# pmeletis/IV2019-boosting-semantic-segmentation-with-weak-labels

Measured on NVIDIA B200. Metric: train_images_per_s, higher is better.
Workload: dtype bf16

## Files before the change

### iv2019-boosting-semantic-segmentation-with-weak-labels_b200/csrc/conv_igemm_sm100.cu

```cuda
#include <cuda.h>

#include <cstdlib>
#include <map>
#include <mutex>
#include <tuple>
#include <vector>

#include "common.cuh"
#include "tc_sm100.cuh"

namespace wlseg {

int check_conv_params(const wlseg_conv_params* p);
int conv_fprop_direct(const wlseg_conv_params* p, const void* x, const void* w, void* y, const float* scale,
                      const float* shift, const void* residual, cudaStream_t s);

constexpr int kBM = 128;
constexpr int kBK = 64;
constexpr int kUmmaK = 16;
constexpr int kEpiWarp0 = 4;
constexpr int kABytes = kBM * kBK * 2;
constexpr int kSmemBudget = 224 * 1024;

struct IgemmParams {
  CUtensorMap map_a;
  CUtensorMap map_b;
  CUtensorMap map_y;
  CUtensorMap map_r;
  void* y;
  const float* scale;
  const float* shift;
  const void* res;
  double* bn_sum;
  double* bn_sqsum;
  const uint32_t* out_mask;
  const float* bnb_scale;
  const float* bnb_shift;
  const float* bnb_mean;
  const float* bnb_invstd;
  wlseg_bn_finalize_args fin;
  CUtensorMap map_ah;
  int halo_rows, halo_bytes, halo_sbo;
  int epi_split;
  int N, P, Q, K, C;
  int R, S, stride, dilation, pad_top, pad_left;
  int y_pitch, res_pitch, res_stride, res_H, res_W;
  int relu;
  int tw_log2;
  int tiles_w, tiles_h, n_tiles, total_tiles;
  int cchunks;
  int num_kb;
  int stages;
  int epi_bufs;
  int res_mid;
  int epi_db;
  int reverse;
  FastDiv fd_n_tiles, fd_tiles_w, fd_tiles_h;
  int m_tiles;
  int units;
};

constexpr int kSubW = 64;
constexpr int kWarpBufBytes = 32 * kSubW * 2;
constexpr int kMaxStages = 8;
constexpr int kMaxEpiWarps = 16;
constexpr int kBarBytes = 512;
constexpr int kSmemMax = 227 * 1024;

template <int BN, bool kPair = false>
struct IgemmCfg {
  static constexpr int kBRows = kPair ? BN / 2 : BN;
  static constexpr int kBBytes = kBRows * kBK * 2;
  static constexpr int kStageBytes = kABytes + kBBytes;
  static constexpr int kTmemCols = 2 * BN < 32 ? 32 : 2 * BN;
};

__device__ __forceinline__ void warp_column_sums(float (&v)[32], int lane) {
#pragma unroll
  for (int off = 16; off >= 1; off >>= 1) {
    const bool upper = (lane & off) != 0;
#pragma unroll
    for (int i = 0; i < off; ++i) {
      const float send = upper ? v[i] : v[i + off];
      const float keep = upper ? v[i + off] : v[i];
      v[i] = keep + __shfl_xor_sync(0xffffffffu, send, off);
    }
  }
}

struct SubTileCursor {
  int tile, st;
  int n, p0, q0, k0;
};

template <int BN, bool kPair>
__device__ __forceinline__ void decode_tile(const IgemmParams& prm, int tile, int rank, int& n, int& p0, int& q0, int& k0) {
  uint32_t umt, unt;
  prm.fd_n_tiles.divmod((uint32_t)tile, umt, unt);
  int mt = (int)umt;
  if (kPair) mt = 2 * mt + rank;
  k0 = (int)unt * BN;
  if (kPair && mt >= prm.m_tiles) {
    n = prm.N; p0 = 0; q0 = 0;
    return;
  }
  if (prm.reverse) mt = prm.m_tiles - 1 - mt;
  uint32_t rest, twi, un, thi;
  prm.fd_tiles_w.divmod((uint32_t)mt, rest, twi);
  prm.fd_tiles_h.divmod(rest, un, thi);
  n = (int)un;
  q0 = (int)twi << prm.tw_log2;
  p0 = (int)thi * (kBM >> prm.tw_log2);
}

template <int BN>
__device__ __forceinline__ int num_subtiles(const IgemmParams& prm, int k0) {
  const int left = prm.K - k0;
  const int full = BN / kSubW;
  const int need = (left + kSubW - 1) / kSubW;
  return need < full ? need : full;
}

template <int BN, typename TY, bool kTmaEpi, int EW, bool kPair, bool kBnb = false, bool kHalo = false>
__global__ void __launch_bounds__(128 + 32 * EW, 1)
conv_igemm_kernel(const __grid_constant__ IgemmParams prm) {
  using Cfg = IgemmCfg<BN, kPair>;
  const uint32_t rank = kPair ? cluster_ctarank() : 0u;
  const int unit0 = kPair ? (int)(blockIdx.x >> 1) : (int)blockIdx.x;
  const int unit_step = kPair ? (int)(gridDim.x >> 1) : (int)gridDim.x;
  constexpr int CG = EW / 4;
  extern __shared__ __align__(1024) uint8_t smem[];
  pdl_launch_dependents();
  if ((smem_u32(smem) & 1023u) != 0) __trap();
  const int stages = prm.stages;
  uint8_t* halo_b = smem + 2 * prm.halo_bytes;
  uint8_t* epi_smem = kHalo ? halo_b + prm.num_kb * Cfg::kBBytes : smem + stages * Cfg::kStageBytes;
  uint64_t* bars = reinterpret_cast<uint64_t*>(epi_smem + prm.epi_bufs * kWarpBufBytes);
  uint64_t* full_bar = bars;
  uint64_t* empty_bar = bars + kMaxStages;
  uint64_t* tfull_bar = bars + 2 * kMaxStages;
  uint64_t* tempty_bar = bars + 2 * kMaxStages + 2;
  uint64_t* rfull_bar = bars + 2 * kMaxStages + 4;
  uint32_t* tmem_slot = reinterpret_cast<uint32_t*>(bars + 2 * kMaxStages + 4 + 2 * kMaxEpiWarps);
  uint64_t* afull_bar = bars + 2 * kMaxStages + 4 + 2 * kMaxEpiWarps + 1;
  uint64_t* aempty_bar = afull_bar + 2;
  uint64_t* bfull_bar = afull_bar + 4;
  float* s_stat = reinterpret_cast<float*>(reinterpret_cast<uint8_t*>(bars) + kBarBytes);

  const int warp = threadIdx.x >> 5;
  const int lane = threadIdx.x & 31;

  if (warp == 0 && lane == 0) {
    tma_prefetch_desc(kHalo ? &prm.map_ah : &prm.map_a);
    tma_prefetch_desc(&prm.map_b);
    if (kTmaEpi) {
      tma_prefetch_desc(&prm.map_y);
      if (prm.res != nullptr) tma_prefetch_desc(&prm.map_r);
    }
  }
  if (warp == 1 && lane == 0) {
    for (int s = 0; s < stages; ++s) {
      mbar_init(smem_u32(full_bar + s), 1);
      mbar_init(smem_u32(empty_bar + s), 1);
    }
    for (int a = 0; a < 2; ++a) {
      mbar_init(smem_u32(tfull_bar + a), 1);
      mbar_init(smem_u32(tempty_bar + a), kPair ? 2 * EW : EW);
    }
    for (int a = 0; a < 2 * EW; ++a) mbar_init(smem_u32(rfull_bar + a), 1);
    if (kHalo) {
      for (int a = 0; a < 2; ++a) { mbar_init(smem_u32(afull_bar + a), 1); mbar_init(smem_u32(aempty_bar + a), 1); }
      mbar_init(smem_u32(bfull_bar), 1);
    }
    fence_barrier_init();
  }
  if (warp == 2) {
    if (kPair) tmem_alloc_pair(smem_u32(tmem_slot), Cfg::kTmemCols);
    else tmem_alloc(smem_u32(tmem_slot), Cfg::kTmemCols);
  }
  if (kTmaEpi && warp == 3 && prm.bn_sum != nullptr)
    for (int j = lane; j < 2 * BN; j += 32) s_stat[j] = 0.f;
  tc_fence_before();
  __syncthreads();
  if (kPair) cluster_sync();
  tc_fence_after();
  const uint32_t tmem_base = *tmem_slot;
  pdl_wait();

  const int TW = 1 << prm.tw_log2;

  if (warp == 0) {
    if (kHalo && lane == 0) {
      mbar_arrive_expect_tx(smem_u32(bfull_bar), prm.num_kb * Cfg::kBBytes);
      for (int kb = 0; kb < prm.num_kb; ++kb)
        tma_load_3d(smem_u32(halo_b + kb * Cfg::kBBytes), &prm.map_b, smem_u32(bfull_bar), 0, kb, 0);
      int it = 0;
      for (int tile = unit0; tile < prm.units; tile += unit_step, ++it) {
        int n, p0, q0, k0;
        decode_tile<BN, kPair>(prm, tile, rank, n, p0, q0, k0);
        const int ab = it & 1;
        mbar_wait(smem_u32(aempty_bar + ab), ((uint32_t)(it >> 1) & 1u) ^ 1u);
        mbar_arrive_expect_tx(smem_u32(afull_bar + ab), prm.halo_bytes);
        tma_load_4d(smem_u32(smem + ab * prm.halo_bytes), &prm.map_ah, smem_u32(afull_bar + ab), 0, q0 - prm.pad_left,
                    p0 - prm.pad_top, n);
      }
    } else if (lane == 0) {
      int stage = 0;
      uint32_t phase = 0;
      for (int tile = unit0; tile < prm.units; tile += unit_step) {
        int n, p0, q0, k0;
// ... 41 lines not shown
        for (int kb = 0; kb < prm.num_kb; ++kb) {
          const uint64_t adesc = make_smem_desc_shifted(a_base + (uint32_t)(r * 2048 + sx * 128), (uint32_t)prm.halo_sbo);
          const uint64_t bdesc = make_smem_desc(smem_u32(halo_b + kb * Cfg::kBBytes));
#pragma unroll
          for (int k = 0; k < kBK / kUmmaK; ++k)
            umma_bf16(d_tmem, adesc + (uint64_t)(k * 2), bdesc + (uint64_t)(k * 2), idesc, (kb | k) != 0);
          if (++sx == prm.S) { sx = 0; ++r; }
        }
        umma_commit(smem_u32(aempty_bar + ab));
        umma_commit(smem_u32(tfull_bar + acc));
      }
    } else if (lane == 0 && rank == 0) {
      constexpr uint32_t idesc = make_idesc(kPair ? 2 * kBM : kBM, BN);
      int stage = 0;
      uint32_t phase = 0;
      int iter = 0;
      for (int tile = unit0; tile < prm.units; tile += unit_step, ++iter) {
        const int acc = iter & 1;
        const uint32_t acc_phase = (iter >> 1) & 1;
        mbar_wait(smem_u32(tempty_bar + acc), acc_phase ^ 1);
        tc_fence_after();
        const uint32_t d_tmem = tmem_base + acc * BN;
        for (int kb = 0; kb < prm.num_kb; ++kb) {
          mbar_wait(smem_u32(full_bar + stage), phase);
          tc_fence_after();
          const uint32_t a_addr = smem_u32(smem + stage * Cfg::kStageBytes);
          const uint64_t adesc = make_smem_desc(a_addr);
          const uint64_t bdesc = make_smem_desc(a_addr + kABytes);
#pragma unroll
          for (int k = 0; k < kBK / kUmmaK; ++k) {
            if (kPair) umma_bf16_pair(d_tmem, adesc + (uint64_t)(k * 2), bdesc + (uint64_t)(k * 2), idesc, (kb | k) != 0);
            else umma_bf16(d_tmem, adesc + (uint64_t)(k * 2), bdesc + (uint64_t)(k * 2), idesc, (kb | k) != 0);
          }
          if (kPair) umma_commit_pair(smem_u32(empty_bar + stage), 3); else umma_commit(smem_u32(empty_bar + stage));
          if (++stage == stages) { stage = 0; phase ^= 1; }
        }
        if (kPair) umma_commit_pair(smem_u32(tfull_bar + acc), 3); else umma_commit(smem_u32(tfull_bar + acc));
      }
    }
  } else if (warp >= kEpiWarp0) {
    const int ew = warp - kEpiWarp0;
    const int quarter = ew & 3;
    const int cgrp = ew >> 2;
    const int et = threadIdx.x - kEpiWarp0 * 32;
    const int row = quarter * 32 + lane;
    const int dy_ = row >> prm.tw_log2, dx_ = row & (TW - 1);
    const uint32_t lane_addr = tmem_base + ((uint32_t)(quarter * 32) << 16);
    auto release_acc = [&](int a) {
      if (kPair) mbar_arrive_cluster(mapa_shared(smem_u32(tempty_bar + a), 0));
      else mbar_arrive(smem_u32(tempty_bar + a));
    };
    int iter = 0;
    if constexpr (kTmaEpi) {
      const bool has_res = prm.res != nullptr;
      const bool has_stat = prm.bn_sum != nullptr;
      const uint32_t sw = (uint32_t)(lane & 7);
      const bool dbuf = has_res || prm.epi_db;
      const bool split = BN == kSubW && prm.epi_split != 0;
      uint8_t* wbuf = epi_smem + ((kHalo && !split) ? quarter : ew) * (kBnb ? 3 : (dbuf ? 2 : 1)) * kWarpBufBytes;
      const int st0 = split ? 0 : cgrp;
      const int st_step = split ? BN / kSubW : CG;
      const int tile0 = unit0 + (split ? cgrp * unit_step : 0);
      const int tile_step = split ? 2 * unit_step : unit_step;
      uint64_t* my_rfull = rfull_bar + 2 * ew;
      const int r0 = quarter * 32;
      const int dy0 = r0 >> prm.tw_log2, dx0 = r0 & (TW - 1);
      constexpr int kResPf = 4;
      struct ResCursor { int tile, st, cnt; };
      ResCursor ld = {tile0, st0, 0}, pf = {tile0, st0, 0};
      auto next_residual = [&](ResCursor& c, bool stage) {
        while (c.tile < prm.units) {
          int n, p0, q0, k0;
          decode_tile<BN, kPair>(prm, c.tile, rank, n, p0, q0, k0);
          if (c.st < num_subtiles<BN>(prm, k0)) {
            const int cx = (q0 + dx0) * prm.res_stride, cy = (p0 + dy0) * prm.res_stride;
            if (stage) {
              const uint32_t bar = smem_u32(my_rfull + (c.cnt & 1));
              mbar_arrive_expect_tx(bar, kWarpBufBytes);
              tma_load_4d(smem_u32(wbuf + (c.cnt & 1) * kWarpBufBytes), &prm.map_r, bar, k0 + c.st * kSubW, cx, cy, n);
            } else {
              tma_prefetch_4d(&prm.map_r, k0 + c.st * kSubW, cx, cy, n);
            }
            ++c.cnt;
            c.st += st_step;
            return;
          }
          c.st = st0;
          c.tile += tile_step;
        }
      };
      if (has_res && lane == 0) {
        for (int i = 0; i < kResPf; ++i) next_residual(pf, false);
        next_residual(ld, true);
      }
      constexpr int kSlots = (BN / kSubW + CG - 1) / CG;
      float a1x[kSlots], a1y[kSlots], a2x[kSlots], a2y[kSlots];
#pragma unroll
      for (int i = 0; i < kSlots; ++i) a1x[i] = a1y[i] = a2x[i] = a2y[i] = 0.f;
      int stat_k0 = -1;
      int cnt = 0;
      float bmx[kSlots], bmy[kSlots], bix[kSlots], biy[kSlots];
#pragma unroll
      for (int i = 0; i < kSlots; ++i) bmx[i] = bmy[i] = bix[i] = biy[i] = 0.f;
      uint2 mcur[kSlots], mnext[kSlots];
      auto load_mask = [&](int tile_, uint2 (&m)[kSlots]) {
#pragma unroll
        for (int i = 0; i < kSlots; ++i) m[i] = make_uint2(0xffffffffu, 0xffffffffu);
        if (prm.out_mask == nullptr || tile_ >= prm.units) return;
        int n_, p0_, q0_, k0_;
        decode_tile<BN, kPair>(prm, tile_, rank, n_, p0_, q0_, k0_);
        const bool ok = (p0_ + dy_ < prm.P) && (q0_ + dx_ < prm.Q) && (n_ < prm.N);
        const int nsub_ = num_subtiles<BN>(prm, k0_);
        const uint2* row = reinterpret_cast<const uint2*>(
            prm.out_mask + (((int64_t)n_ * prm.P + p0_ + dy_) * prm.Q + q0_ + dx_) * (prm.K >> 5) + (k0_ >> 5));
#pragma unroll
        for (int i = 0; i < kSlots; ++i) {
          const int st_ = st0 + i * st_step;
          m[i] = (ok && st_ < nsub_) ? __ldg(row + st_) : make_uint2(0u, 0u);
        }
      };
      load_mask(unit0, mnext);
      for (int tile = unit0; tile < prm.units; tile += unit_step, ++iter) {
        int n, p0, q0, k0;
        decode_tile<BN, kPair>(prm, tile, rank, n, p0, q0, k0);
        const bool valid = (p0 + dy_ < prm.P) && (q0 + dx_ < prm.Q) && (n < prm.N);
#pragma unroll
        for (int i = 0; i < kSlots; ++i) mcur[i] = mnext[i];
        load_mask(tile + unit_step, mnext);
        const int acc = iter & 1;
        const uint32_t acc_phase = (iter >> 1) & 1;
        const int nsub = num_subtiles<BN>(prm, k0);
        if (has_stat) {
          if (stat_k0 >= 0 && k0 != stat_k0) __trap();
          if constexpr (kBnb) {
            if (stat_k0 < 0) {
#pragma unroll
              for (int i = 0; i < kSlots; ++i) {
                const int c = k0 + (st0 + i * st_step) * kSubW + 2 * lane;
                if (c + 1 < prm.K) {
                  bmx[i] = __ldg(prm.bnb_mean + c); bmy[i] = __ldg(prm.bnb_mean + c + 1);
                  bix[i] = __ldg(prm.bnb_invstd + c); biy[i] = __ldg(prm.bnb_invstd + c + 1);
                }
              }
            }
          }
          stat_k0 = k0;
        }
        mbar_wait(smem_u32(tfull_bar + acc), acc_phase);
        tc_fence_after();
        const bool idle = split ? ((iter & 1) != cgrp) : (cgrp >= nsub);
        if (idle) {
          tc_fence_before();
          __syncwarp();
          if (lane == 0) release_acc(acc);
        }
#pragma unroll
        for (int slot = 0; slot < kSlots; ++slot) {
          const int st = st0 + slot * st_step;
          if (st >= nsub || idle) break;
          if constexpr (kBnb) {
            uint8_t* zb = wbuf + (cnt & 1) * kWarpBufBytes;
            uint8_t* ob = wbuf + 2 * kWarpBufBytes;
            if (lane == 0) {
              bulk_wait_read<0>();
              next_residual(ld, true);
              next_residual(pf, false);
            }
            __syncwarp();
            mbar_wait(smem_u32(my_rfull + (cnt & 1)), (uint32_t)((cnt >> 1) & 1));
#pragma unroll
            for (int half = 0; half < 2; ++half) {
              const int col = st * kSubW + half * 32;
              uint32_t v[32];
              tmem_ld<32>(lane_addr + (uint32_t)(acc * BN + col), v);
              tmem_ld_wait();
              if (half == 1 && st + CG >= nsub) {
                tc_fence_before();
                __syncwarp();
// ... 4 lines not shown
              for (int j = 0; j < 32; ++j) f[j] = valid ? __uint_as_float(v[j]) : 0.f;
              uint4 raw[4];
#pragma unroll
              for (int g = 0; g < 4; ++g)
                raw[g] = *reinterpret_cast<const uint4*>(zb + lane * 128 + ((((uint32_t)(half * 4 + g)) ^ sw) << 4));
              const float4* sc4 = reinterpret_cast<const float4*>(prm.bnb_scale + k0 + col);
              const float4* sh4 = reinterpret_cast<const float4*>(prm.bnb_shift + k0 + col);
              uint4 outv[4];
#pragma unroll
              for (int g = 0; g < 4; ++g) {
                const __nv_bfloat162* hz = reinterpret_cast<const __nv_bfloat162*>(&raw[g]);
                __nv_bfloat162* ho = reinterpret_cast<__nv_bfloat162*>(&outv[g]);
                const float4 sca = __ldg(sc4 + 2 * g), scb = __ldg(sc4 + 2 * g + 1);
                const float4 sha = __ldg(sh4 + 2 * g), shb = __ldg(sh4 + 2 * g + 1);
                const float scs[8] = {sca.x, sca.y, sca.z, sca.w, scb.x, scb.y, scb.z, scb.w};
                const float shs[8] = {sha.x, sha.y, sha.z, sha.w, shb.x, shb.y, shb.z, shb.w};
#pragma unroll
                for (int e = 0; e < 4; ++e) {
                  const float2 zz = __bfloat1622float2(hz[e]);
                  const float gx = fmaf(zz.x, scs[2 * e], shs[2 * e]) > 0.f ? f[g * 8 + 2 * e] : 0.f;
                  const float gy = fmaf(zz.y, scs[2 * e + 1], shs[2 * e + 1]) > 0.f ? f[g * 8 + 2 * e + 1] : 0.f;
                  ho[e] = __floats2bfloat162_rn(gx, gy);
                }
              }
#pragma unroll
              for (int g = 0; g < 4; ++g)
                *reinterpret_cast<uint4*>(ob + lane * 128 + ((((uint32_t)(half * 4 + g)) ^ sw) << 4)) = outv[g];
            }
            fence_async_smem();
            __syncwarp();
            if (lane == 0) {
              tma_store_4d(&prm.map_y, smem_u32(ob), k0 + st * kSubW, q0 + dx0, p0 + dy0, n);
              bulk_commit();
            }
            {
              const uint32_t coff = (uint32_t)((lane & 3) << 2);
              float s0x = 0.f, s0y = 0.f, s1x = 0.f, s1y = 0.f;
              const float mx = bmx[slot], my = bmy[slot], ix = bix[slot], iy = biy[slot];
#pragma unroll
              for (int r = 0; r < 32; ++r) {
                const uint32_t o = (uint32_t)(r * 128) + ((((uint32_t)(lane >> 2)) ^ (uint32_t)(r & 7)) << 4) + coff;
                const float2 g2 = __bfloat1622float2(*reinterpret_cast<const __nv_bfloat162*>(ob + o));
                const float2 z2 = __bfloat1622float2(*reinterpret_cast<const __nv_bfloat162*>(zb + o));
                s0x += g2.x * (z2.x - mx) * ix; s0y += g2.y * (z2.y - my) * iy;
                s1x += g2.x; s1y += g2.y;
              }
              a1x[slot] += s0x; a1y[slot] += s0y; a2x[slot] += s1x; a2y[slot] += s1y;
            }
            __syncwarp();
            ++cnt;
            continue;
          }
          uint8_t* buf = wbuf + (dbuf ? (cnt & 1) * kWarpBufBytes : 0);
          const bool mid = has_res && prm.res_mid;
          if (lane == 0 && !mid) {
            if (!has_res && dbuf) bulk_wait_read<1>(); else bulk_wait_read<0>();
            if (has_res) {
              next_residual(ld, true);
              next_residual(pf, false);
            }
          }
          __syncwarp();
          if (has_res && !mid) mbar_wait(smem_u32(my_rfull + (cnt & 1)), (uint32_t)((cnt >> 1) & 1));
          uint8_t* myrow = buf + lane * 128;
#pragma unroll
          for (int half = 0; half < 2; ++half) {
            const int col = st * kSubW + half * 32;
            if (mid && half == 1) {
              if (lane == 0) {
                bulk_wait_read<0>();
                next_residual(ld, true);
                next_residual(pf, false);
              }
              __syncwarp();
            }
            const uint32_t mword = half == 0 ? mcur[slot].x : mcur[slot].y;
            uint32_t v[32];
            tmem_ld<32>(lane_addr + (uint32_t)(acc * BN + col), v);
            tmem_ld_wait();
            if (half == 1 && st + CG >= nsub) {
              tc_fence_before();
              __syncwarp();
              if (lane == 0) release_acc(acc);
            }
            float f[32];
#pragma unroll
            for (int j = 0; j < 32; ++j) f[j] = __uint_as_float(v[j]);
            if (prm.scale != nullptr) {
              const float4* sc4 = reinterpret_cast<const float4*>(prm.scale + k0 + col);
              const float4* sh4 = reinterpret_cast<const float4*>(prm.shift + k0 + col);
#pragma unroll
              for (int g = 0; g < 8; ++g) {
                const float4 sc = __ldg(sc4 + g);
                const float4 sh = __ldg(sh4 + g);
                f[g * 4 + 0] = fmaf(f[g * 4 + 0], sc.x, sh.x);
                f[g * 4 + 1] = fmaf(f[g * 4 + 1], sc.y, sh.y);
                f[g * 4 + 2] = fmaf(f[g * 4 + 2], sc.z, sh.z);
                f[g * 4 + 3] = fmaf(f[g * 4 + 3], sc.w, sh.w);
              }
            }
            uint4* slot4[4];
#pragma unroll
            for (int g = 0; g < 4; ++g)
              slot4[g] = reinterpret_cast<uint4*>(myrow + ((((uint32_t)(half * 4 + g)) ^ sw) << 4));
            if (mid && half == 0) mbar_wait(smem_u32(my_rfull + (cnt & 1)), (uint32_t)((cnt >> 1) & 1));
            if (has_res) {
              uint4 raw[4];
#pragma unroll
              for (int g = 0; g < 4; ++g) raw[g] = *slot4[g];
#pragma unroll
              for (int g = 0; g < 4; ++g) {
                const __nv_bfloat162* h = reinterpret_cast<const __nv_bfloat162*>(&raw[g]);
#pragma unroll
                for (int e = 0; e < 4; ++e) {
                  const float2 t = __bfloat1622float2(h[e]);
                  f[g * 8 + 2 * e] += t.x;
                  f[g * 8 + 2 * e + 1] += t.y;
                }
              }
            }
            if (prm.out_mask != nullptr) {
#pragma unroll
              for (int j = 0; j < 32; ++j) f[j] = ((mword >> j) & 1u) ? f[j] : 0.f;
            }
            if (has_stat && !valid) {
#pragma unroll
              for (int j = 0; j < 32; ++j) f[j] = 0.f;
            }
            uint4 outv[4];
            if (prm.relu) {
#pragma unroll
              for (int g = 0; g < 4; ++g) {
                __nv_bfloat162* ho = reinterpret_cast<__nv_bfloat162*>(&outv[g]);
#pragma unroll
                for (int e = 0; e < 4; ++e) {
                  uint32_t packed;
                  asm("cvt.rn.relu.bf16x2.f32 %0, %1, %2;" : "=r"(packed) : "f"(f[g * 8 + 2 * e + 1]), "f"(f[g * 8 + 2 * e]));
                  reinterpret_cast<uint32_t*>(ho)[e] = packed;
                }
              }
            } else {
#pragma unroll
              for (int g = 0; g < 4; ++g) {
                __nv_bfloat162* ho = reinterpret_cast<__nv_bfloat162*>(&outv[g]);
#pragma unroll
                for (int e = 0; e < 4; ++e) ho[e] = __floats2bfloat162_rn(f[g * 8 + 2 * e], f[g * 8 + 2 * e + 1]);
              }
            }
#pragma unroll
            for (int g = 0; g < 4; ++g) *slot4[g] = outv[g];
          }
          fence_async_smem();
          __syncwarp();
          if (lane == 0) {
            tma_store_4d(&prm.map_y, smem_u32(buf), k0 + st * kSubW, q0 + dx0, p0 + dy0, n);
            bulk_commit();
          }
          if (has_stat) {
            const uint8_t* base = buf + ((lane & 3) << 2);
            float s1x = 0.f, s1y = 0.f, s2x = 0.f, s2y = 0.f;
#pragma unroll
            for (int r = 0; r < 32; ++r) {
              const __nv_bfloat162 h = *reinterpret_cast<const __nv_bfloat162*>(
                  base + r * 128 + ((((uint32_t)(lane >> 2)) ^ (uint32_t)(r & 7)) << 4));
              const float2 t = __bfloat1622float2(h);
              s1x += t.x; s1y += t.y;
              s2x = fmaf(t.x, t.x, s2x); s2y = fmaf(t.y, t.y, s2y);
            }
            a1x[slot] += s1x; a1y[slot] += s1y; a2x[slot] += s2x; a2y[slot] += s2y;
          }
          ++cnt;
        }
      }
      if (has_stat) {
        constexpr int kBufsPerWarp = kBnb ? 3 : 0;
        const int nbuf = kBufsPerWarp ? kBufsPerWarp : (dbuf ? 2 : 1);
        if (lane == 0) bulk_wait_read<0>();
        __syncwarp();
        float* park = reinterpret_cast<float*>(wbuf);
#pragma unroll
        for (int i = 0; i < kSlots; ++i) {
          if (kHalo && !split && cgrp != 0) break;
          park[(i * 2 + 0) * kSubW + 2 * lane] = a1x[i]; park[(i * 2 + 0) * kSubW + 2 * lane + 1] = a1y[i];
          park[(i * 2 + 1) * kSubW + 2 * lane] = a2x[i]; park[(i * 2 + 1) * kSubW + 2 * lane + 1] = a2y[i];
        }
        epi_barrier<32 * EW>();
        if (stat_k0 >= 0) {
          for (int j = et; j < BN; j += 32 * EW) {
            if (stat_k0 + j < prm.K) {
              const int st = j / kSubW, ch = j % kSubW;
              const int cg = split ? 0 : st % CG, i = split ? 0 : st / CG;
              float t1 = 0.f, t2 = 0.f;
              for (int g2 = 0; g2 < (split ? CG : 1); ++g2) {
#pragma unroll
                for (int q4 = 0; q4 < 4; ++q4) {
                  const float* src = reinterpret_cast<const float*>(epi_smem + (q4 + 4 * (cg + g2)) * nbuf * kWarpBufBytes);
                  t1 += src[(i * 2 + 0) * kSubW + ch];
                  t2 += src[(i * 2 + 1) * kSubW + ch];
                }
              }
              atomicAdd(prm.bn_sum + stat_k0 + j, (double)t1);
              atomicAdd(prm.bn_sqsum + stat_k0 + j, (double)t2);
            }
          }
        }
      }
      if constexpr (!kBnb) {
        if (has_stat && prm.fin.counter != nullptr) {
          uint32_t* s_last = tmem_slot + 1;
          __threadfence();
          epi_barrier<32 * EW>();
          if (et == 0) *s_last = (atomicAdd(prm.fin.counter, 1u) == gridDim.x - 1) ? 1u : 0u;
          epi_barrier<32 * EW>();
          if (*s_last != 0u) {
            __threadfence();
            const double nn = (double)prm.fin.count;
            for (int c = et; c < prm.K; c += 32 * EW) {
              const double m = __ldcg(prm.bn_sum + c) / nn;
              double var = __ldcg(prm.bn_sqsum + c) / nn - m * m;
              if (var < 0.0) var = 0.0;
              const float mf = (float)m, vf = (float)var;
// ... 170 lines not shown
  return 0;
}

static int pick_bn(int K) { return K > 128 ? 256 : (K > 64 ? 128 : (K > 32 ? 64 : 32)); }

static bool igemm_supported(const wlseg_conv_params* p) {
  if (p->dtype != WLSEG_BF16) return false;
  if (p->stride != 1 && p->stride != 2) return false;
  if (p->C % 8 != 0 || p->x_pitch % 8 != 0) return false;
  if (p->R * p->S > 64 || p->dilation > 64) return false;
  if (p->N > 65535) return false;
  return true;
}

template <typename K>
static int max_active_pairs(K kernel, int threads, int smem_bytes) {
  cudaLaunchConfig_t cfg = {};
  cfg.gridDim = dim3(2 * kNumSMs);
  cfg.blockDim = dim3(threads);
  cfg.dynamicSmemBytes = smem_bytes;
  cudaLaunchAttribute attr[1];
  attr[0].id = cudaLaunchAttributeClusterDimension;
  attr[0].val.clusterDim.x = 2; attr[0].val.clusterDim.y = 1; attr[0].val.clusterDim.z = 1;
  cfg.attrs = attr;
  cfg.numAttrs = 1;
  int n = 0;
  if (cudaOccupancyMaxActiveClusters(&n, kernel, &cfg) != cudaSuccess) { cudaGetLastError(); return 0; }
  return n;
}

template <typename... KArgs, typename... Args>
static cudaError_t launch_pair(void (*kernel)(KArgs...), int clusters, int threads, size_t smem, cudaStream_t stream,
                               Args&&... args) {
  cudaLaunchConfig_t cfg = {};
  cfg.gridDim = dim3(2 * clusters);
  cfg.blockDim = dim3(threads);
  cfg.dynamicSmemBytes = smem;
  cfg.stream = stream;
  cudaLaunchAttribute attr[2];
  attr[0].id = cudaLaunchAttributeClusterDimension;
  attr[0].val.clusterDim.x = 2; attr[0].val.clusterDim.y = 1; attr[0].val.clusterDim.z = 1;
  attr[1].id = cudaLaunchAttributeProgrammaticStreamSerialization;
  attr[1].val.programmaticStreamSerializationAllowed = 1;
  cfg.attrs = attr;
  cfg.numAttrs = pdl_enabled() ? 2 : 1;
  return cudaLaunchKernelEx(&cfg, kernel, static_cast<KArgs>(args)...);
}

static int halo_smem_bytes(const IgemmParams& prm, int bn, int bufs_per_warp, int warps = 4) {
  return 2 * prm.halo_bytes + prm.num_kb * bn * kBK * 2 + warps * bufs_per_warp * kWarpBufBytes + kBarBytes + 2 * bn * 4;
}
static bool epi_split_enabled() { return env_int("WLSEG_EPI_SPLIT", 1) != 0; }

template <int BN, typename TY, bool kTmaEpi, int EW, bool kPair = false, bool kBnb = false, bool kHalo = false>
static int launch_igemm_ew(IgemmParams& prm, cudaStream_t s) {
  using Cfg = IgemmCfg<BN, kPair>;
  static_assert(!kBnb || kTmaEpi, "the BN-backward form lives in the staged epilogue");
  static_assert(!kHalo || (kTmaEpi && !kPair && BN == 64), "the halo form: staged epilogue, single CTA, BN = 64");
  static bool configured = false;
  if (!configured) {
    WLSEG_CUDA(cudaFuncSetAttribute(conv_igemm_kernel<BN, TY, kTmaEpi, EW, kPair, kBnb, kHalo>,
                                    cudaFuncAttributeMaxDynamicSharedMemorySize, kSmemMax));
    configured = true;
  }
  if constexpr (kHalo) {
    prm.epi_db = 0;
    prm.res_mid = getenv("WLSEG_RES_MID") != nullptr ? atoi(getenv("WLSEG_RES_MID")) : 1;
    const int bufs = kBnb ? 3 : (prm.res != nullptr ? 2 : 1);
    prm.epi_split = (epi_split_enabled() && halo_smem_bytes(prm, BN, bufs, 8) <= kSmemMax) ? 1 : 0;
    const int ewarps = prm.epi_split ? 8 : 4;
    prm.epi_bufs = ewarps * bufs;
    prm.stages = 0;
    const int smem_bytes = halo_smem_bytes(prm, BN, bufs, ewarps);
    WLSEG_CHECK_ARG(smem_bytes <= kSmemMax, "conv(tcgen05, halo): shared memory plan does not fit");
    prm.units = prm.total_tiles;
    int grid = prm.total_tiles < conv_sms() ? prm.total_tiles : conv_sms();
    WLSEG_CUDA(launch_pdl(conv_igemm_kernel<BN, TY, kTmaEpi, EW, false, kBnb, true>, dim3(grid), dim3(128 + 32 * EW), smem_bytes,
                          s, prm));
    return 0;
  }
  const int db_env = getenv("WLSEG_EPI_DB") != nullptr ? atoi(getenv("WLSEG_EPI_DB")) : -1;
  prm.epi_db = (kTmaEpi && !kBnb && prm.res == nullptr && prm.R * prm.S == 1 &&
                (db_env >= 0 ? db_env != 0 : prm.num_kb <= 8)) ? 1 : 0;
  prm.epi_bufs = kTmaEpi ? (kBnb ? 3 * EW : ((prm.res != nullptr || prm.epi_db) ? 2 * EW : EW)) : 0;
  prm.epi_split = (kTmaEpi && BN == kSubW && epi_split_enabled()) ? 1 : 0;
  prm.res_mid = getenv("WLSEG_RES_MID") != nullptr ? atoi(getenv("WLSEG_RES_MID")) : 1;
  const int fixed = prm.epi_bufs * kWarpBufBytes + kBarBytes + (kTmaEpi ? 2 * BN * 4 : 0);
  int stages = (kSmemMax - fixed) / Cfg::kStageBytes;
  if (stages > kMaxStages) stages = kMaxStages;
  WLSEG_CHECK_ARG(stages >= 2, "conv(tcgen05): shared memory plan leaves fewer than 2 pipeline stages");
  prm.stages = stages;
  const int smem_bytes = stages * Cfg::kStageBytes + fixed;
  if constexpr (kPair) {
    static int max_pairs = -1;
    if (max_pairs < 0) max_pairs = max_active_pairs(conv_igemm_kernel<BN, TY, kTmaEpi, EW, true, kBnb>, 128 + 32 * EW, kSmemMax);
    WLSEG_CHECK_ARG(max_pairs > 0, "conv(tcgen05): the device cannot host a CTA pair of this kernel");
    prm.units = (int)ceil_div(prm.m_tiles, 2) * prm.n_tiles;
    int clusters = prm.units < max_pairs ? prm.units : max_pairs;
    if (clusters > conv_sms() / 2) clusters = conv_sms() / 2;
    if (prm.bn_sum != nullptr && clusters % prm.n_tiles != 0) clusters -= clusters % prm.n_tiles;
    WLSEG_CHECK_ARG(clusters > 0, "conv(tcgen05): no CTA pair fits the N-tile constraint of the fused statistics");
    WLSEG_CUDA(launch_pair(conv_igemm_kernel<BN, TY, kTmaEpi, EW, true, kBnb>, clusters, 128 + 32 * EW, smem_bytes, s, prm));
    return 0;
  }
  prm.units = prm.total_tiles;
  int grid = prm.total_tiles < conv_sms() ? prm.total_tiles : conv_sms();
  if (kTmaEpi && prm.bn_sum != nullptr && grid % prm.n_tiles != 0) grid -= grid % prm.n_tiles;
  WLSEG_CHECK_ARG(grid > 0, "conv(tcgen05): no CTA fits the N-tile constraint of the fused statistics");
  WLSEG_CUDA(launch_pdl(conv_igemm_kernel<BN, TY, kTmaEpi, EW, false, kBnb>, dim3(grid), dim3(128 + 32 * EW), smem_bytes, s, prm));
  return 0;
}

template <int BN, typename TY, bool kTmaEpi>
static int launch_igemm(IgemmParams& prm, cudaStream_t s) {
  return launch_igemm_ew<BN, TY, kTmaEpi, 8>(prm, s);
}

static int pair_mode() {
  const char* e = getenv("WLSEG_PAIR");
  return e != nullptr ? atoi(e) : -1;
}

struct BnbArgs { const float* scale; const float* shift; const float* mean; const float* invstd; };

static int conv_fprop_igemm(const wlseg_conv_params* p, const void* x, const void* w, void* y, const float* scale,
                            const float* shift, const void* residual, double* bn_sum, double* bn_sqsum,
                            cudaStream_t s, const uint32_t* out_mask = nullptr, const BnbArgs* bnb = nullptr,
                            const wlseg_bn_finalize_args* fin = nullptr) {
  WLSEG_CHECK_ARG((((uintptr_t)x) & 15) == 0 && (((uintptr_t)w) & 15) == 0, "conv(tcgen05): x / w must be 16-byte aligned");
  IgemmParams prm;
  const int BN = pick_bn(p->K);
  int tw_log2 = 4;
  if (p->Q <= 8) tw_log2 = 3;
  if (p->Q <= 4) tw_log2 = 2;
  if (p->P == 1) tw_log2 = 7;
  const bool halo_shape = BN == 64 && p->C == 64 && p->K == 64 && p->stride == 1 && p->dilation == 1 &&
                          (p->S == 1 || p->S == 3) && p->R * p->S <= 9 && p->R * p->S > 1 && p->W >= 16 && p->Q >= 16 &&
                          p->P > 1 && p->y_dtype != WLSEG_F32 && env_int("WLSEG_HALO", 1) != 0;
  if (halo_shape) tw_log2 = p->S == 1 ? 4 : 3;
  const int TW = 1 << tw_log2, TH = kBM / TW;
  WLSEG_CHECK_ARG(TW * p->stride <= 256 && TH * p->stride <= 256, "conv(tcgen05): TMA box too large");
  {
    uint64_t dims[4] = {(uint64_t)p->C, (uint64_t)p->W, (uint64_t)p->H, (uint64_t)p->N};
    uint64_t strides[3] = {(uint64_t)p->x_pitch * 2, (uint64_t)p->x_pitch * 2 * p->W,
                           (uint64_t)p->x_pitch * 2 * p->W * p->H};
    uint32_t box[4] = {(uint32_t)kBK, (uint32_t)(TW * p->stride), (uint32_t)(TH * p->stride), 1};
    uint32_t estr[4] = {1, (uint32_t)p->stride, (uint32_t)p->stride, 1};
    if (int e = encode_tensor_map(&prm.map_a, x, 2, 4, dims, strides, box, estr, 0)) return e;
  }
  const bool f32out = (p->y_dtype == WLSEG_F32);
  bool tma_epi = !f32out && BN >= kSubW && (p->K % kSubW == 0) && (p->y_pitch % 8 == 0) &&
                 ((((uintptr_t)y) & 15) == 0) && ((((uintptr_t)scale) & 15) == 0) && ((((uintptr_t)shift) & 15) == 0);
  const int bw = TW < 32 ? TW : 32, bh = 32 / bw;
  if (residual != nullptr && ((p->res_pitch % 8 != 0) || ((((uintptr_t)residual) & 15) != 0) ||
                              bw * p->res_stride > 256 || bh * p->res_stride > 256))
    tma_epi = false;
  bool use_pair = false;
  if (BN == 256 && tma_epi) {
    const int mode = pair_mode();
    const int kblocks = p->R * p->S * (int)ceil_div(p->C, kBK);
    const bool pair_default = residual != nullptr ? kblocks >= 8 : kblocks >= 2;
    use_pair = (mode == 1) || (mode == -1 && pair_default);
    if (bnb != nullptr) use_pair = true;
  }
  WLSEG_CHECK_ARG(bnb == nullptr || (tma_epi && residual != nullptr && BN >= kSubW && p->res_stride == 1 &&
                                     bn_sum != nullptr && bn_sqsum != nullptr && scale == nullptr && p->relu == 0),
                  "conv_fprop_bnbwd: needs the staged bf16 epilogue (K %% 64 == 0, 16-byte aligned y / z, pitches %% 8 == 0)");
  bool use_halo = false;
// ... 25 lines not shown
      uint64_t dims[4] = {(uint64_t)p->K, (uint64_t)p->Q, (uint64_t)p->P, (uint64_t)p->N};
      uint64_t strides[3] = {(uint64_t)p->y_pitch * 2, (uint64_t)p->y_pitch * 2 * p->Q,
                             (uint64_t)p->y_pitch * 2 * p->Q * p->P};
      uint32_t box[4] = {(uint32_t)kSubW, (uint32_t)bw, (uint32_t)bh, 1};
      uint32_t estr[4] = {1, 1, 1, 1};
      if (int e = encode_tensor_map(&prm.map_y, y, 2, 4, dims, strides, box, estr, 2)) return e;
    }
    if (residual != nullptr) {
      const int rs = p->res_stride;
      uint64_t dims[4] = {(uint64_t)p->K, (uint64_t)p->res_W, (uint64_t)p->res_H, (uint64_t)p->N};
      uint64_t strides[3] = {(uint64_t)p->res_pitch * 2, (uint64_t)p->res_pitch * 2 * p->res_W,
                             (uint64_t)p->res_pitch * 2 * p->res_W * p->res_H};
      uint32_t box[4] = {(uint32_t)kSubW, (uint32_t)(bw * rs), (uint32_t)(bh * rs), 1};
      uint32_t estr[4] = {1, (uint32_t)rs, (uint32_t)rs, 1};
      if (int e = encode_tensor_map(&prm.map_r, residual, 2, 4, dims, strides, box, estr, 3)) return e;
    }
  }
  prm.y = y; prm.scale = scale; prm.shift = shift; prm.res = residual;
  prm.bn_sum = bn_sum; prm.bn_sqsum = bn_sqsum;
  prm.out_mask = out_mask;
  prm.bnb_scale = prm.bnb_shift = prm.bnb_mean = prm.bnb_invstd = nullptr;
  prm.fin = wlseg_bn_finalize_args{};
  if (fin != nullptr) {
    WLSEG_CHECK_ARG(tma_epi && bn_sum != nullptr && bnb == nullptr && !pdl_enabled(),
                    "conv_fprop_bn: needs the staged bf16 epilogue (K %% 64 == 0, aligned y) and no programmatic launches");
    prm.fin = *fin;
  }
  if (bnb != nullptr) {
    prm.bnb_scale = bnb->scale; prm.bnb_shift = bnb->shift; prm.bnb_mean = bnb->mean; prm.bnb_invstd = bnb->invstd;
  }
  WLSEG_CHECK_ARG(out_mask == nullptr || (tma_epi && p->K % 32 == 0 && (((uintptr_t)out_mask) & 3) == 0),
                  "conv_fprop_masked: needs the staged bf16 epilogue (K %% 64 == 0, aligned tensors)");
  prm.N = p->N; prm.P = p->P; prm.Q = p->Q; prm.K = p->K; prm.C = p->C;
  prm.R = p->R; prm.S = p->S; prm.stride = p->stride; prm.dilation = p->dilation;
  prm.pad_top = p->pad_top; prm.pad_left = p->pad_left;
  prm.y_pitch = p->y_pitch; prm.res_pitch = p->res_pitch; prm.res_stride = p->res_stride;
  prm.res_H = p->res_H; prm.res_W = p->res_W;
  prm.relu = p->relu;
  prm.reverse = p->reverse ? 1 : 0;
  prm.tw_log2 = tw_log2;
  prm.tiles_w = (int)ceil_div(p->Q, TW);
  prm.tiles_h = (int)ceil_div(p->P, TH);
  prm.n_tiles = (int)ceil_div(p->K, BN);
  const int64_t total = (int64_t)p->N * prm.tiles_h * prm.tiles_w * prm.n_tiles;
  WLSEG_CHECK_ARG(total < ((int64_t)1 << 31), "conv(tcgen05): too many tiles");
  prm.total_tiles = (int)total;
  prm.m_tiles = (int)(total / prm.n_tiles);
  prm.fd_n_tiles = make_fastdiv((uint32_t)prm.n_tiles);
  prm.fd_tiles_w = make_fastdiv((uint32_t)prm.tiles_w);
  prm.fd_tiles_h = make_fastdiv((uint32_t)prm.tiles_h);
  prm.units = prm.total_tiles;
  prm.cchunks = (int)ceil_div(p->C, kBK);
  prm.num_kb = p->R * p->S * prm.cchunks;
#define WLSEG_IGEMM_CASE(bn)                                                          \
  case bn:                                                                            \
    if (f32out) return launch_igemm<bn, float, false>(prm, s);                        \
    if (bn >= kSubW && tma_epi) return launch_igemm<bn, __nv_bfloat16, (bn >= kSubW)>(prm, s); \
    return launch_igemm<bn, __nv_bfloat16, false>(prm, s);
  if (use_halo) {
    if (bnb != nullptr) return launch_igemm_ew<64, __nv_bfloat16, true, 8, false, true, true>(prm, s);
    return launch_igemm_ew<64, __nv_bfloat16, true, 8, false, false, true>(prm, s);
  }
  if (bnb != nullptr) {
    if (BN == 256) return launch_igemm_ew<256, __nv_bfloat16, true, 8, true, true>(prm, s);
    if (BN == 128) return launch_igemm_ew<128, __nv_bfloat16, true, 8, false, true>(prm, s);
    return launch_igemm_ew<64, __nv_bfloat16, true, 8, false, true>(prm, s);
  }
  if (use_pair) return launch_igemm_ew<256, __nv_bfloat16, true, 8, true>(prm, s);
  switch (BN) {
    WLSEG_IGEMM_CASE(32)
    WLSEG_IGEMM_CASE(64)
    WLSEG_IGEMM_CASE(128)
    WLSEG_IGEMM_CASE(256)
  }
#undef WLSEG_IGEMM_CASE
  WLSEG_CHECK_ARG(false, "conv(tcgen05): internal tile selection error");
}

}

using namespace wlseg;

extern "C" int wlseg_conv2d_tcgen05_supported(const wlseg_conv_params* p) {
  if (p == nullptr) return 0;
  return igemm_supported(p) ? 1 : 0;
}

extern "C" int wlseg_conv2d_fprop_masked(const wlseg_conv_params* p, const void* x, const void* w, void* y,
                                         const void* residual, const uint8_t* out_mask, wlseg_stream_t stream) {
  if (int e = check_conv_params(p)) return e;
  if (p->N == 0) return 0;
  WLSEG_CHECK_ARG(x && w && y && out_mask, "conv_fprop_masked: null pointer");
  WLSEG_CHECK_ARG(igemm_supported(p) && p->y_dtype == WLSEG_BF16 && p->relu == 0,
                  "conv_fprop_masked: tcgen05 bf16 configurations without ReLU only");
  if (residual != nullptr)
    WLSEG_CHECK_ARG(p->res_stride > 0 && p->res_pitch >= p->K && (p->P - 1) * p->res_stride < p->res_H &&
                        (p->Q - 1) * p->res_stride < p->res_W,
                    "conv_fprop_masked: residual geometry inconsistent");
  return conv_fprop_igemm(p, x, w, y, nullptr, nullptr, residual, nullptr, nullptr, (cudaStream_t)stream,
                          reinterpret_cast<const uint32_t*>(out_mask));
}

extern "C" int wlseg_conv2d_fprop_bnbwd(const wlseg_conv_params* p, const void* x, const void* w, void* y, const void* z,
                                        const float* scale, const float* shift, const float* mean, const float* invstd,
                                        double* dgamma, double* dbeta, wlseg_stream_t stream) {
  if (int e = check_conv_params(p)) return e;
  if (p->N == 0) return 0;
  WLSEG_CHECK_ARG(x && w && y && z && scale && shift && mean && invstd && dgamma && dbeta, "conv_fprop_bnbwd: null pointer");
  WLSEG_CHECK_ARG(igemm_supported(p) && p->y_dtype == WLSEG_BF16 && p->relu == 0 && p->K % 64 == 0,
                  "conv_fprop_bnbwd: tcgen05 bf16 configurations with K %% 64 == 0 and without ReLU only");
  WLSEG_CHECK_ARG(p->res_stride == 1 && p->res_pitch >= p->K && p->res_H == p->P && p->res_W == p->Q,
                  "conv_fprop_bnbwd: z must have the output's shape (res_* fields of the parameters describe it)");
  WLSEG_CHECK_ARG(((((uintptr_t)scale) | ((uintptr_t)shift)) & 15) == 0, "conv_fprop_bnbwd: scale / shift must be 16-byte aligned");
  const BnbArgs bnb = {scale, shift, mean, invstd};
  return conv_fprop_igemm(p, x, w, y, nullptr, nullptr, z, dgamma, dbeta, (cudaStream_t)stream, nullptr, &bnb);
}

extern "C" int wlseg_conv2d_fprop_bn(const wlseg_conv_params* p, const void* x, const void* w, void* y, double* bn_sum,
                                     double* bn_sqsum, const wlseg_bn_finalize_args* fin, wlseg_stream_t stream) {
  if (int e = check_conv_params(p)) return e;
  if (p->N == 0) return 0;
// ... 32 lines not shown
```

Baseline: 379.4.

## Specialize staged conv epilogue on compile-time residual/stat forms and use fused bf16 adds

```diff
diff --git a/iv2019-boosting-semantic-segmentation-with-weak-labels_b200/csrc/conv_igemm_sm100.cu b/iv2019-boosting-semantic-segmentation-with-weak-labels_b200/csrc/conv_igemm_sm100.cu
--- a/iv2019-boosting-semantic-segmentation-with-weak-labels_b200/csrc/conv_igemm_sm100.cu
+++ b/iv2019-boosting-semantic-segmentation-with-weak-labels_b200/csrc/conv_igemm_sm100.cu
@@ -52,13 +52,16 @@
   int num_kb;
   int stages;
   int epi_bufs;
-  int res_mid;
   int epi_db;
   int reverse;
   FastDiv fd_n_tiles, fd_tiles_w, fd_tiles_h;
   int m_tiles;
   int units;
 };
+
+constexpr int kFormRes = 1;
+constexpr int kFormStat = 2;
+constexpr int kFormBnb = 4 | kFormRes | kFormStat;
 
 constexpr int kSubW = 64;
 constexpr int kWarpBufBytes = 32 * kSubW * 2;
@@ -86,6 +89,18 @@
       v[i] = keep + __shfl_xor_sync(0xffffffffu, send, off);
     }
   }
+}
+
+__device__ __forceinline__ void add_bf16x2(float& x, float& y, uint32_t packed) {
+  asm("{\n\t.reg .b16 lo, hi;\n\tmov.b32 {lo, hi}, %2;\n\t"
+      "add.rn.f32.bf16 %0, lo, %0;\n\tadd.rn.f32.bf16 %1, hi, %1;\n\t}"
+      : "+f"(x), "+f"(y) : "r"(packed));
+}
+__device__ __forceinline__ void stat_bf16x2(float& s1x, float& s1y, float& s2x, float& s2y, uint32_t packed) {
+  asm("{\n\t.reg .b16 lo, hi;\n\tmov.b32 {lo, hi}, %4;\n\t"
+      "add.rn.f32.bf16 %0, lo, %0;\n\tadd.rn.f32.bf16 %1, hi, %1;\n\t"
+      "fma.rn.f32.bf16 %2, lo, lo, %2;\n\tfma.rn.f32.bf16 %3, hi, hi, %3;\n\t}"
+      : "+f"(s1x), "+f"(s1y), "+f"(s2x), "+f"(s2y) : "r"(packed));
 }
 
 struct SubTileCursor {
@@ -121,10 +136,11 @@
   return need < full ? need : full;
 }
 
-template <int BN, typename TY, bool kTmaEpi, int EW, bool kPair, bool kBnb = false, bool kHalo = false>
+template <int BN, typename TY, bool kTmaEpi, int EW, bool kPair, int kForm = 0, bool kHalo = false>
 __global__ void __launch_bounds__(128 + 32 * EW, 1)
 conv_igemm_kernel(const __grid_constant__ IgemmParams prm) {
   using Cfg = IgemmCfg<BN, kPair>;
+  constexpr bool kBnb = (kForm & kFormBnb) == kFormBnb;
   const uint32_t rank = kPair ? cluster_ctarank() : 0u;
   const int unit0 = kPair ? (int)(blockIdx.x >> 1) : (int)blockIdx.x;
   const int unit_step = kPair ? (int)(gridDim.x >> 1) : (int)gridDim.x;
@@ -155,7 +171,7 @@
     tma_prefetch_desc(&prm.map_b);
     if (kTmaEpi) {
       tma_prefetch_desc(&prm.map_y);
-      if (prm.res != nullptr) tma_prefetch_desc(&prm.map_r);
+      if (kForm & kFormRes) tma_prefetch_desc(&prm.map_r);
     }
   }
   if (warp == 1 && lane == 0) {
@@ -303,8 +319,8 @@
     };
     int iter = 0;
     if constexpr (kTmaEpi) {
-      const bool has_res = prm.res != nullptr;
-      const bool has_stat = prm.bn_sum != nullptr;
+      constexpr bool has_res = (kForm & kFormRes) != 0;
+      constexpr bool has_stat = (kForm & kFormStat) != 0;
       const uint32_t sw = (uint32_t)(lane & 7);
       const bool dbuf = has_res || prm.epi_db;
       const bool split = BN == kSubW && prm.epi_split != 0;
@@ -375,6 +391,7 @@
         int n, p0, q0, k0;
         decode_tile<BN, kPair>(prm, tile, rank, n, p0, q0, k0);
         const bool valid = (p0 + dy_ < prm.P) && (q0 + dx_ < prm.Q) && (n < prm.N);
+        const bool edge = has_stat && !__all_sync(0xffffffffu, valid);
 #pragma unroll
         for (int i = 0; i < kSlots; ++i) mcur[i] = mnext[i];
         load_mask(tile + unit_step, mnext);
@@ -485,21 +502,17 @@
             continue;
           }
           uint8_t* buf = wbuf + (dbuf ? (cnt & 1) * kWarpBufBytes : 0);
-          const bool mid = has_res && prm.res_mid;
-          if (lane == 0 && !mid) {
-            if (!has_res && dbuf) bulk_wait_read<1>(); else bulk_wait_read<0>();
-            if (has_res) {
-              next_residual(ld, true);
-              next_residual(pf, false);
+          if constexpr (!has_res) {
+            if (lane == 0) {
+              if (dbuf) bulk_wait_read<1>(); else bulk_wait_read<0>();
             }
           }
           __syncwarp();
-          if (has_res && !mid) mbar_wait(smem_u32(my_rfull + (cnt & 1)), (uint32_t)((cnt >> 1) & 1));
           uint8_t* myrow = buf + lane * 128;
 #pragma unroll
           for (int half = 0; half < 2; ++half) {
             const int col = st * kSubW + half * 32;
-            if (mid && half == 1) {
+            if (has_res && half == 1) {
               if (lane == 0) {
                 bulk_wait_read<0>();
                 next_residual(ld, true);
@@ -536,29 +549,21 @@
 #pragma unroll
             for (int g = 0; g < 4; ++g)
               slot4[g] = reinterpret_cast<uint4*>(myrow + ((((uint32_t)(half * 4 + g)) ^ sw) << 4));
-            if (mid && half == 0) mbar_wait(smem_u32(my_rfull + (cnt & 1)), (uint32_t)((cnt >> 1) & 1));
-            if (has_res) {
+            if (has_res && half == 0) mbar_wait(smem_u32(my_rfull + (cnt & 1)), (uint32_t)((cnt >> 1) & 1));
+            if constexpr (has_res) {
               uint4 raw[4];
 #pragma unroll
               for (int g = 0; g < 4; ++g) raw[g] = *slot4[g];
 #pragma unroll
               for (int g = 0; g < 4; ++g) {
-                const __nv_bfloat162* h = reinterpret_cast<const __nv_bfloat162*>(&raw[g]);
-#pragma unroll
-                for (int e = 0; e < 4; ++e) {
-                  const float2 t = __bfloat1622float2(h[e]);
-                  f[g * 8 + 2 * e] += t.x;
-                  f[g * 8 + 2 * e + 1] += t.y;
-                }
+                const uint32_t* h = reinterpret_cast<const uint32_t*>(&raw[g]);
+#pragma unroll
+                for (int e = 0; e < 4; ++e) add_bf16x2(f[g * 8 + 2 * e], f[g * 8 + 2 * e + 1], h[e]);
               }
             }
             if (prm.out_mask != nullptr) {
 #pragma unroll
               for (int j = 0; j < 32; ++j) f[j] = ((mword >> j) & 1u) ? f[j] : 0.f;
-            }
-            if (has_stat && !valid) {
-#pragma unroll
-              for (int j = 0; j < 32; ++j) f[j] = 0.f;
             }
             uint4 outv[4];
             if (prm.relu) {
@@ -582,6 +587,10 @@
             }
 #pragma unroll
             for (int g = 0; g < 4; ++g) *slot4[g] = outv[g];
+            if (has_stat && edge && !valid) {
+#pragma unroll
+              for (int g = 0; g < 4; ++g) *slot4[g] = make_uint4(0u, 0u, 0u, 0u);
+            }
           }
           fence_async_smem();
           __syncwarp();
@@ -593,13 +602,9 @@
             const uint8_t* base = buf + ((lane & 3) << 2);
             float s1x = 0.f, s1y = 0.f, s2x = 0.f, s2y = 0.f;
 #pragma unroll
-            for (int r = 0; r < 32; ++r) {
-              const __nv_bfloat162 h = *reinterpret_cast<const __nv_bfloat162*>(
-                  base + r * 128 + ((((uint32_t)(lane >> 2)) ^ (uint32_t)(r & 7)) << 4));
-              const float2 t = __bfloat1622float2(h);
-              s1x += t.x; s1y += t.y;
-              s2x = fmaf(t.x, t.x, s2x); s2y = fmaf(t.y, t.y, s2y);
-            }
+            for (int r = 0; r < 32; ++r)
+              stat_bf16x2(s1x, s1y, s2x, s2y, *reinterpret_cast<const uint32_t*>(
+                                                  base + r * 128 + ((((uint32_t)(lane >> 2)) ^ (uint32_t)(r & 7)) << 4)));
             a1x[slot] += s1x; a1y[slot] += s1y; a2x[slot] += s2x; a2y[slot] += s2y;
           }
           ++cnt;
@@ -876,20 +881,20 @@
 }
 static bool epi_split_enabled() { return env_int("WLSEG_EPI_SPLIT", 1) != 0; }
 
-template <int BN, typename TY, bool kTmaEpi, int EW, bool kPair = false, bool kBnb = false, bool kHalo = false>
+template <int BN, typename TY, bool kTmaEpi, int EW, bool kPair = false, int kForm = 0, bool kHalo = false>
 static int launch_igemm_ew(IgemmParams& prm, cudaStream_t s) {
   using Cfg = IgemmCfg<BN, kPair>;
-  static_assert(!kBnb || kTmaEpi, "the BN-backward form lives in the staged epilogue");
+  constexpr bool kBnb = (kForm & kFormBnb) == kFormBnb;
+  static_assert(kForm == 0 || kTmaEpi, "the epilogue forms live in the staged epilogue");
   static_assert(!kHalo || (kTmaEpi && !kPair && BN == 64), "the halo form: staged epilogue, single CTA, BN = 64");
   static bool configured = false;
   if (!configured) {
-    WLSEG_CUDA(cudaFuncSetAttribute(conv_igemm_kernel<BN, TY, kTmaEpi, EW, kPair, kBnb, kHalo>,
+    WLSEG_CUDA(cudaFuncSetAttribute(conv_igemm_kernel<BN, TY, kTmaEpi, EW, kPair, kForm, kHalo>,
                                     cudaFuncAttributeMaxDynamicSharedMemorySize, kSmemMax));
     configured = true;
   }
   if constexpr (kHalo) {
     prm.epi_db = 0;
-    prm.res_mid = getenv("WLSEG_RES_MID") != nullptr ? atoi(getenv("WLSEG_RES_MID")) : 1;
     const int bufs = kBnb ? 3 : (prm.res != nullptr ? 2 : 1);
     prm.epi_split = (epi_split_enabled() && halo_smem_bytes(prm, BN, bufs, 8) <= kSmemMax) ? 1 : 0;
     const int ewarps = prm.epi_split ? 8 : 4;
@@ -899,16 +904,14 @@
     WLSEG_CHECK_ARG(smem_bytes <= kSmemMax, "conv(tcgen05, halo): shared memory plan does not fit");
     prm.units = prm.total_tiles;
     int grid = prm.total_tiles < conv_sms() ? prm.total_tiles : conv_sms();
-    WLSEG_CUDA(launch_pdl(conv_igemm_kernel<BN, TY, kTmaEpi, EW, false, kBnb, true>, dim3(grid), dim3(128 + 32 * EW), smem_bytes,
+    WLSEG_CUDA(launch_pdl(conv_igemm_kernel<BN, TY, kTmaEpi, EW, false, kForm, true>, dim3(grid), dim3(128 + 32 * EW), smem_bytes,
                           s, prm));
     return 0;
   }
-  const int db_env = getenv("WLSEG_EPI_DB") != nullptr ? atoi(getenv("WLSEG_EPI_DB")) : -1;
   prm.epi_db = (kTmaEpi && !kBnb && prm.res == nullptr && prm.R * prm.S == 1 &&
-                (db_env >= 0 ? db_env != 0 : prm.num_kb <= 8)) ? 1 : 0;
+                prm.num_kb <= 8) ? 1 : 0;
   prm.epi_bufs = kTmaEpi ? (kBnb ? 3 * EW : ((prm.res != nullptr || prm.epi_db) ? 2 * EW : EW)) : 0;
   prm.epi_split = (kTmaEpi && BN == kSubW && epi_split_enabled()) ? 1 : 0;
-  prm.res_mid = getenv("WLSEG_RES_MID") != nullptr ? atoi(getenv("WLSEG_RES_MID")) : 1;
   const int fixed = prm.epi_bufs * kWarpBufBytes + kBarBytes + (kTmaEpi ? 2 * BN * 4 : 0);
   int stages = (kSmemMax - fixed) / Cfg::kStageBytes;
   if (stages > kMaxStages) stages = kMaxStages;
@@ -917,27 +920,39 @@
   const int smem_bytes = stages * Cfg::kStageBytes + fixed;
   if constexpr (kPair) {
     static int max_pairs = -1;
-    if (max_pairs < 0) max_pairs = max_active_pairs(conv_igemm_kernel<BN, TY, kTmaEpi, EW, true, kBnb>, 128 + 32 * EW, kSmemMax);
+    if (max_pairs < 0) max_pairs = max_active_pairs(conv_igemm_kernel<BN, TY, kTmaEpi, EW, true, kForm>, 128 + 32 * EW, kSmemMax);
     WLSEG_CHECK_ARG(max_pairs > 0, "conv(tcgen05): the device cannot host a CTA pair of this kernel");
     prm.units = (int)ceil_div(prm.m_tiles, 2) * prm.n_tiles;
     int clusters = prm.units < max_pairs ? prm.units : max_pairs;
     if (clusters > conv_sms() / 2) clusters = conv_sms() / 2;
     if (prm.bn_sum != nullptr && clusters % prm.n_tiles != 0) clusters -= clusters % prm.n_tiles;
     WLSEG_CHECK_ARG(clusters > 0, "conv(tcgen05): no CTA pair fits the N-tile constraint of the fused statistics");
-    WLSEG_CUDA(launch_pair(conv_igemm_kernel<BN, TY, kTmaEpi, EW, true, kBnb>, clusters, 128 + 32 * EW, smem_bytes, s, prm));
+    WLSEG_CUDA(launch_pair(conv_igemm_kernel<BN, TY, kTmaEpi, EW, true, kForm>, clusters, 128 + 32 * EW, smem_bytes, s, prm));
     return 0;
   }
   prm.units = prm.total_tiles;
   int grid = prm.total_tiles < conv_sms() ? prm.total_tiles : conv_sms();
   if (kTmaEpi && prm.bn_sum != nullptr && grid % prm.n_tiles != 0) grid -= grid % prm.n_tiles;
   WLSEG_CHECK_ARG(grid > 0, "conv(tcgen05): no CTA fits the N-tile constraint of the fused statistics");
-  WLSEG_CUDA(launch_pdl(conv_igemm_kernel<BN, TY, kTmaEpi, EW, false, kBnb>, dim3(grid), dim3(128 + 32 * EW), smem_bytes, s, prm));
+  WLSEG_CUDA(launch_pdl(conv_igemm_kernel<BN, TY, kTmaEpi, EW, false, kForm>, dim3(grid), dim3(128 + 32 * EW), smem_bytes, s, prm));
   return 0;
 }
 
-template <int BN, typename TY, bool kTmaEpi>
+template <int BN, typename TY>
 static int launch_igemm(IgemmParams& prm, cudaStream_t s) {
-  return launch_igemm_ew<BN, TY, kTmaEpi, 8>(prm, s);
+  return launch_igemm_ew<BN, TY, false, 8>(prm, s);
+}
+
+template <int BN, bool kPair = false, bool kHalo = false>
+static int launch_staged(IgemmParams& prm, int form, cudaStream_t s) {
+  switch (form) {
+    case 0: return launch_igemm_ew<BN, __nv_bfloat16, true, 8, kPair, 0, kHalo>(prm, s);
+    case kFormRes: return launch_igemm_ew<BN, __nv_bfloat16, true, 8, kPair, kFormRes, kHalo>(prm, s);
+    case kFormStat: return launch_igemm_ew<BN, __nv_bfloat16, true, 8, kPair, kFormStat, kHalo>(prm, s);
+    case kFormRes | kFormStat: return launch_igemm_ew<BN, __nv_bfloat16, true, 8, kPair, kFormRes | kFormStat, kHalo>(prm, s);
+    case kFormBnb: return launch_igemm_ew<BN, __nv_bfloat16, true, 8, kPair, kFormBnb, kHalo>(prm, s);
+  }
+  WLSEG_CHECK_ARG(false, "conv(tcgen05): unknown epilogue form %d", form);
 }
 
 static int pair_mode() {
@@ -1069,21 +1084,18 @@
   prm.units = prm.total_tiles;
   prm.cchunks = (int)ceil_div(p->C, kBK);
   prm.num_kb = p->R * p->S * prm.cchunks;
-#define WLSEG_IGEMM_CASE(bn)                                                          \
-  case bn:                                                                            \
-    if (f32out) return launch_igemm<bn, float, false>(prm, s);                        \
-    if (bn >= kSubW && tma_epi) return launch_igemm<bn, __nv_bfloat16, (bn >= kSubW)>(prm, s); \
-    return launch_igemm<bn, __nv_bfloat16, false>(prm, s);
-  if (use_halo) {
-    if (bnb != nullptr) return launch_igemm_ew<64, __nv_bfloat16, true, 8, false, true, true>(prm, s);
-    return launch_igemm_ew<64, __nv_bfloat16, true, 8, false, false, true>(prm, s);
-  }
-  if (bnb != nullptr) {
-    if (BN == 256) return launch_igemm_ew<256, __nv_bfloat16, true, 8, true, true>(prm, s);
-    if (BN == 128) return launch_igemm_ew<128, __nv_bfloat16, true, 8, false, true>(prm, s);
-    return launch_igemm_ew<64, __nv_bfloat16, true, 8, false, true>(prm, s);
-  }
-  if (use_pair) return launch_igemm_ew<256, __nv_bfloat16, true, 8, true>(prm, s);
+  if (tma_epi) {
+    const int form = bnb != nullptr ? kFormBnb : (residual != nullptr ? kFormRes : 0) | (bn_sum != nullptr ? kFormStat : 0);
+    if (use_halo) return launch_staged<64, false, true>(prm, form, s);
+    if (use_pair) return launch_staged<256, true>(prm, form, s);
+    if (BN == 256) return launch_staged<256>(prm, form, s);
+    if (BN == 128) return launch_staged<128>(prm, form, s);
+    if (BN == 64) return launch_staged<64>(prm, form, s);
+  }
+#define WLSEG_IGEMM_CASE(bn)                                               \
+  case bn:                                                                 \
+    if (f32out) return launch_igemm<bn, float>(prm, s);                    \
+    return launch_igemm<bn, __nv_bfloat16>(prm, s);
   switch (BN) {
     WLSEG_IGEMM_CASE(32)
     WLSEG_IGEMM_CASE(64)
```

Measured after the change: 389.4 (median of 6 runs). 2.6% higher.
